# anisanazim/Movie-Recommendation-Engine

Measured on AMD Instinct MI355X. Metric: item embeddings/sec + top-K ANN queries/sec, ML-25M d=256, 1/2/4/8 GPU, higher is better.
Workload: dtype f64 cdf / f32 features / fp4 sign planes (exact integer Hamming); 1 GPU; SYN-25M (ML-25M-shaped: U=162541 M=59047 R=25000095), F=128 H=256 d=256, 2 GCN layers, W=100 L=2 T=10, LSH 512-bit, 10000 queries K=11, rng=numpy (the reference's np.random MT19937 stream generated on device: neighbour ids bit-exact with the reference CPU path); global_items=59047, queries=10000, parallelism=item-shard x1

## Files before the change

include/pinsage_hip.h:

```cpp
#ifndef PINSAGE_HIP_H
#define PINSAGE_HIP_H

#include <stddef.h>
#include <stdint.h>

#ifdef __cplusplus
extern "C" {
#endif

#define PS_OK 0
#define PS_EINVAL (-1)
#define PS_ELAUNCH (-2)
#define PS_EWORKSPACE (-3)
#define PS_EUNSUPPORTED (-4)

#define PS_RNG_STREAM 0
#define PS_RNG_PHILOX 1
#define PS_RNG_STREAM_RAW 2

#define PS_RNG_STREAM_WALKS 3

#define PS_WALK_HALF_BUCKETS 0x100

typedef void *ps_stream_t;

int ps_abi_version(void);
const char *ps_error_string(int code);

size_t ps_csr_build_workspace_bytes(int64_t E, int64_t V);
int ps_csr_build(const int64_t *src, const int64_t *dst, const float *w, int64_t E, int64_t V,
                 int64_t *rowptr, int32_t *col, double *wsorted,
                 void *workspace, size_t workspace_bytes, ps_stream_t stream);

int ps_cdf_build(const int64_t *rowptr, const double *wsorted, int64_t V, double *cdf, ps_stream_t stream);

int ps_guide_build(const int64_t *rowptr, const double *cdf, int64_t V, uint32_t *nodeinfo, int32_t *guide,
                   ps_stream_t stream);

int ps_pack_edges(const int32_t *col, const double *cdf, const int32_t *guide, int64_t E, void *packed,
                  ps_stream_t stream);

int ps_bucket_build(const int64_t *rowptr, const int32_t *col, const double *cdf, const int32_t *guide, int64_t V,
                    int64_t E, void *buckets, ps_stream_t stream);

int ps_bucket_build_half(const int64_t *rowptr, const int32_t *col, const double *cdf, const int32_t *guide, int64_t V,
                         int64_t E, void *buckets, ps_stream_t stream);

int ps_dest_info_build(const int32_t *col, const uint32_t *nodeinfo, int64_t E, int64_t V, void *dest_info, ps_stream_t stream);

int ps_graph_stats(const int64_t *rowptr, const int32_t *col, int64_t E, int64_t V, int64_t *flags,
                   ps_stream_t stream);

int ps_walk_sample(const int64_t *rowptr, const int32_t *col, const double *cdf, int64_t V,
                   const int64_t *starts, int64_t B, int W, int L, int T,
                   int rng_mode, const double *uniforms, const int64_t *uoff,
                   uint64_t seed, uint32_t call, const uint32_t *nodeinfo, const int32_t *guide,
                   const void *packed, const void *buckets, const void *dest_info,
                   int32_t *ids, int32_t *counts, int32_t *nvalid, ps_stream_t stream);

int ps_walk_sample_layers(const int64_t *rowptr, const int32_t *col, const double *cdf, int64_t V,
                          const int64_t *starts, int64_t B, int W, int L, int T,
                          int rng_mode, const double *uniforms, const int64_t *uoff, int64_t layer_stride,
                          uint64_t seed, uint32_t call, const uint32_t *nodeinfo, const int32_t *guide,
                          const void *packed, const void *buckets, const void *dest_info, int layers,
                          int32_t *ids, int32_t *counts, int32_t *nvalid, ps_stream_t stream);

int ps_walk_paths(const int64_t *rowptr, const int32_t *col, const double *cdf, int64_t V,
                  const int64_t *starts, int64_t B, int L, int rng_mode, const double *uniforms,
                  const int64_t *uoff, uint64_t seed, uint32_t call, int walk_mod,
                  const uint32_t *nodeinfo, const int32_t *guide, int32_t *paths, ps_stream_t stream);

int ps_uniform_offsets(const int64_t *rowptr, int64_t V, const int64_t *starts, int64_t B, int W, int L,
                       int64_t *uoff, int64_t *total, ps_stream_t stream);

int ps_mt19937_chunk_log2(void);
int ps_mt19937_window_shift(void);
int ps_mt19937_raw_stream(const uint32_t *state_in, int pos_in, int64_t n, uint32_t *raw, uint32_t *state_out,
                          int32_t *pos_out, const uint32_t *jump_polys, int jump_levels, const uint32_t *radix_polys,
                          int radix_levels, const uint32_t *window_polys, int n_window, const int64_t *ranges,
                          int n_ranges, void *workspace, size_t workspace_bytes, ps_stream_t stream);
size_t ps_mt19937_workspace_bytes(int64_t skip, int64_t n);
int ps_mt19937_random_sample(const uint32_t *state_in, int pos_in, int64_t skip, int64_t n, double *out,
                             uint32_t *state_out, int32_t *pos_out, const uint32_t *jump_polys, int jump_levels,
                             const uint32_t *radix_polys, int radix_levels, const uint32_t *window_polys, int n_window,
                             void *workspace, size_t workspace_bytes, ps_stream_t stream);

int ps_importance_pool(const float *x, int64_t N, int H, const int32_t *ids, const int32_t *counts,
                       const float *wts, const int32_t *nvalid, int64_t B, int T, int64_t max_idx,
                       int renorm, float *out, ps_stream_t stream);

#define PS_RELU 1
#define PS_L2NORM 2
#define PS_WPERM 4
int ps_permute_k(const float *W, int64_t rows, int K, int ld, float *out, ps_stream_t stream);
int ps_linear(const float *x, int64_t M, int K, const float *W, int ldw, const float *b, int N,
              const float *x2, int K2, const float *W2, int ldw2, int flags, float *y, ps_stream_t stream);

size_t ps_gcn_layer_workspace_bytes(int64_t M, int H);
int ps_gcn_layer(const float *x, int64_t M, int K, const float *W, int ldw, const float *b, int N, const float *h_full,
                 int64_t n_full, int H, const int32_t *ids, const int32_t *counts, const float *wts, const int32_t *nvalid,
                 int T, int64_t max_idx, int renorm, const float *W2, int ldw2, int flags, float *y, void *workspace,
                 size_t workspace_bytes, ps_stream_t stream);

int ps_lsh_encode(const float *x, int64_t N, int D, const float *A, int nbits, uint8_t *codes, int flags, ps_stream_t stream);

size_t ps_hamming_topk_workspace_bytes(int64_t nq, int64_t N, int cs, int k);
int ps_hamming_topk(const uint8_t *qcodes, int64_t nq, const uint8_t *codes, int64_t N, int cs, int k,
                    int64_t id_offset, int32_t *dist, int64_t *ids,
                    void *workspace, size_t workspace_bytes, ps_stream_t stream);

size_t ps_lsh_planes_bytes(int64_t n, int cs);
int ps_lsh_expand(const uint8_t *codes, int64_t n, int cs, void *planes, ps_stream_t stream);
size_t ps_hamming_topk_mfma_workspace_bytes(int64_t nq, int64_t N, int cs, int k);
int ps_hamming_topk_mfma(const void *qplanes, int64_t nq, const void *dbplanes, int64_t N, int cs, int k,
                         int64_t id_offset, int32_t *dist, int64_t *ids,
                         void *workspace, size_t workspace_bytes, ps_stream_t stream);
int ps_hamming_topk_mfma_codes(const uint8_t *qcodes, int64_t nq, const void *dbplanes, int64_t N, int cs, int k,
                               int64_t id_offset, int32_t *dist, int64_t *ids,
                               void *workspace, size_t workspace_bytes, ps_stream_t stream);

int ps_topk_merge(const int32_t *dist_in, const int64_t *ids_in, int P, int64_t nq, int k,
                  int32_t *dist, int64_t *ids, ps_stream_t stream);
int ps_topk_merge_strided(const int32_t *dist_in, int64_t dist_stride, const int64_t *ids_in, int64_t ids_stride,
                          int P, int64_t nq, int k, int32_t *dist, int64_t *ids, ps_stream_t stream);

size_t ps_dot_topk_workspace_bytes(int64_t nq, int64_t N, int D, int k);
int ps_dot_topk(const float *E, int64_t N, int D, const int64_t *qidx, int64_t nq, int k, int exclude_self,
                float *vals, int64_t *ids, void *workspace, size_t workspace_bytes, ps_stream_t stream);

int ps_row_dot(const float *A, int64_t nA, const float *B, int64_t nB, int D, const int64_t *ia, const int64_t *ib, int64_t n,
               float *out, ps_stream_t stream);
int ps_rank_count(const float *E, int64_t N, int D, int64_t id_offset, const float *Q, int64_t nq, const float *thr,
                  const int64_t *tid, int64_t *count, ps_stream_t stream);

size_t ps_l2_topk_workspace_bytes(int64_t nq, int64_t N, int D, int k);
int ps_l2_topk(const float *X, int64_t N, int D, const float *Q, int64_t nq, int k, const int32_t *assign,
               const uint32_t *probe, int words, float *dist, int64_t *ids, void *workspace,
               size_t workspace_bytes, ps_stream_t stream);

size_t ps_ivf_topk_workspace_bytes(int64_t nq, int64_t N, int D, int k, int nlist, int nprobe, int64_t max_list);
int ps_ivf_topk(const float *X, int64_t N, int D, const int64_t *list_ptr, int nlist, int64_t max_list,
                const int64_t *item_ids, const float *Q, int64_t nq, const int32_t *probes, int nprobe, int k,
                float *dist, int64_t *ids, void *workspace, size_t workspace_bytes, ps_stream_t stream);

int ps_spmm_csr(const int64_t *rowptr, const int32_t *col, const float *val, const float *x, int64_t N, int H,
                int64_t V, int64_t E, float *out, ps_stream_t stream);

#define PS_COOC_WINDOW 512
typedef struct {
    int32_t a, b, count, window;
} ps_cooc_record;
size_t ps_cooc_planes_bytes(int64_t U, int64_t M, int max_mult);
int ps_cooc_planes(const int32_t *user, const int32_t *item, const int32_t *mult, int64_t n, int64_t U, int64_t M,
                   int max_mult, void *planes, size_t planes_bytes, int64_t *item_stats, int32_t *max_seen, ps_stream_t stream);
int ps_cooc_pairs(const void *planes, int64_t U, int64_t M, int max_mult, int64_t max_sq, const int64_t *item_stats, int64_t thr,
                  ps_cooc_record *records, int64_t capacity, int64_t *count, int64_t *h_count, ps_stream_t stream);
int ps_cooc_keys(const ps_cooc_record *records, int64_t n, int64_t U, int64_t M, const int64_t *iptr, const int32_t *iuser,
                 const int32_t *imult, const int64_t *uptr, const int32_t *uitem, const int32_t *upos, int64_t R,
                 int64_t *keys, ps_stream_t stream);
int ps_cooc_emit(const ps_cooc_record *records, const int64_t *perm, int64_t n, int64_t *edge_index, float *edge_weight,
                 ps_stream_t stream);

#define PS_HN_PER_QUERY 1
#define PS_HN_EXCLUDE_DIAG 2
#define PS_LOSS_SHARED 0
#define PS_LOSS_PER_QUERY 1
#define PS_LOSS_BATCH_HARD 2
int ps_hardest_negative(const float *Q, int64_t B, int D, const float *X, int64_t N, int flags, uint64_t *best, float *sim,
                        int64_t *idx, ps_stream_t stream);
int ps_margin_loss(const float *Q, const float *P, int64_t B, int D, const uint64_t *best, float margin, float *row_loss,
                   int64_t *idx, uint8_t *active, float *loss, ps_stream_t stream);
int ps_margin_loss_bwd(const float *Q, const float *P, const float *X, int64_t B, int64_t N, int D, int mode, const int64_t *idx,
                       const uint8_t *active, const float *grad_out, float *dQ, float *dP, float *dX, ps_stream_t stream);

#ifdef __cplusplus
}
#endif
#endif
```

movie-recommendation-engine_amd/pinsage_hip/dense.py:

```python
from __future__ import annotations

import os

import torch

from . import native as nv


def _rowmajor(w):
    if w.dtype != torch.float32:
        raise TypeError("fp32 expected")
    if w.dim() != 2:
        raise ValueError("2-D matrix expected")
    if w.stride(1) != 1 or w.stride(0) < w.size(1):
        w = w.contiguous()
    return w, int(w.stride(0)) if w.size(0) > 1 else max(int(w.stride(0)), int(w.size(1)))


def _require_cuda(*tensors):
    for t in tensors:
        if t is not None and not t.is_cuda:
            raise nv.NativeError("libpinsage_hip takes device (HBM) tensors; got a CPU tensor (no CPU fallback)")


def _ptr_view(t):
    if t is None:
        return nv.C.c_void_p(0)
    if not t.is_cuda:
        raise nv.NativeError("device tensor expected")
    return nv.C.c_void_p(t.data_ptr())


class StagedWeight:
    __slots__ = ("t", "shape")

    def __init__(self, t):
        self.t = t
        self.shape = t.shape

    def size(self, i):
        return self.t.size(i)


def stage_weight(W):
    if isinstance(W, StagedWeight) or W is None:
        return W
    _require_cuda(W)
    if W.dim() != 2 or W.dtype != torch.float32 or int(W.size(1)) % 32 != 0:
        return W
    Wk, ld = _rowmajor(W)
    out = torch.empty((int(Wk.size(0)), int(Wk.size(1))), dtype=torch.float32, device=W.device)
    with torch.cuda.device(W.device):
        nv.call("ps_permute_k", _ptr_view(Wk), nv.i64(int(Wk.size(0))), nv.i32(int(Wk.size(1))), nv.i32(ld), nv.ptr(out), nv.stream())
    return StagedWeight(out)


def linear(x, W, b=None, x2=None, W2=None, relu=False, l2norm=False):
    staged = isinstance(W, StagedWeight)
    if x2 is not None and isinstance(W2, StagedWeight) != staged:
        raise ValueError("W and W2 must both be staged or both plain")
    if staged:
        W, W2 = W.t, (W2.t if W2 is not None else None)
    _require_cuda(x, W, b, x2, W2)
    x = x.contiguous()
    if x.dtype != torch.float32:
        raise TypeError("fp32 expected")
    M, K = int(x.size(0)), int(x.size(1))
    Wk, ldw = _rowmajor(W)
    N = int(Wk.size(0))
    if int(Wk.size(1)) != K:
        raise ValueError(f"shape mismatch: x [{M},{K}] vs W {tuple(Wk.shape)}")
    K2, ldw2, W2k = 0, 0, None
    if x2 is not None:
        x2 = x2.contiguous()
        W2k, ldw2 = _rowmajor(W2)
        K2 = int(x2.size(1))
        if int(W2k.size(1)) != K2 or int(W2k.size(0)) != N or int(x2.size(0)) != M:
            raise ValueError("shape mismatch in the second operand pair")
    if b is not None:
        b = b.contiguous()
    y = torch.empty((M, N), dtype=torch.float32, device=x.device)
    flags = (nv.PS_RELU if relu else 0) | (nv.PS_L2NORM if l2norm else 0) | (nv.PS_WPERM if staged else 0)
    with torch.cuda.device(x.device):
        nv.call("ps_linear", nv.ptr(x), nv.i64(M), nv.i32(K), _ptr_view(Wk), nv.i32(ldw), nv.ptr(b), nv.i32(N),
                                    nv.ptr(x2), nv.i32(K2), _ptr_view(W2k), nv.i32(ldw2), nv.i32(flags), nv.ptr(y),
                                    nv.stream())
    return y


def gcn_layer(x, W, b, h_full, ids, counts, nvalid, W2, wts=None, max_idx=None, renorm=True, relu=True, l2norm=True):
    from . import sampling
    staged = isinstance(W, StagedWeight)
    if isinstance(W2, StagedWeight) != staged:
        raise ValueError("W and W2 must both be staged or both plain")
    Wm, W2m = (W.t, W2.t) if staged else (W, W2)
    _require_cuda(x, Wm, b, h_full, W2m, ids, counts, wts, nvalid)
    x, h_full = x.contiguous(), h_full.contiguous()
    if x.dtype != torch.float32 or h_full.dtype != torch.float32:
        raise TypeError("fp32 expected")
    M, K = int(x.size(0)), int(x.size(1))
    n_full, H = int(h_full.size(0)), int(h_full.size(1))
    Wk, ldw = _rowmajor(Wm)
    W2k, ldw2 = _rowmajor(W2m)
    N = int(Wk.size(0))
    if int(Wk.size(1)) != K or int(W2k.size(1)) != H or int(W2k.size(0)) != N or int(ids.size(0)) != M:
        raise ValueError("shape mismatch")
    T = int(ids.size(1))
    if max_idx is None:
        max_idx = n_full - 1
    if b is not None:
        b = b.contiguous()
    ids, nvalid = ids.contiguous(), nvalid.contiguous()
    counts = counts.contiguous() if counts is not None else None
    wts = wts.contiguous() if wts is not None else None
    flags = (nv.PS_RELU if relu else 0) | (nv.PS_L2NORM if l2norm else 0) | (nv.PS_WPERM if staged else 0)
    L = nv.lib()
    wsb = int(L.ps_gcn_layer_workspace_bytes(nv.i64(M), nv.i32(H)))
    if wsb > 0:
        y = torch.empty((M, N), dtype=torch.float32, device=x.device)
        ws = torch.empty((wsb,), dtype=torch.uint8, device=x.device)
        with torch.cuda.device(x.device):
            rc = L.ps_gcn_layer(nv.ptr(x), nv.i64(M), nv.i32(K), _ptr_view(Wk), nv.i32(ldw), nv.ptr(b), nv.i32(N), nv.ptr(h_full),
                                nv.i64(n_full), nv.i32(H), nv.ptr(ids), nv.ptr(counts), nv.ptr(wts), nv.ptr(nvalid), nv.i32(T),
                                nv.i64(int(max_idx)), nv.i32(int(renorm)), _ptr_view(W2k), nv.i32(ldw2), nv.i32(flags), nv.ptr(y),
                                nv.ptr(ws), nv.C.c_size_t(wsb), nv.stream())
        if rc != nv.PS_EUNSUPPORTED:
            nv.check(rc, "ps_gcn_layer")
            return y
    h_neigh = sampling.importance_pool(h_full, ids=ids, counts=counts, wts=wts, nvalid=nvalid, max_idx=max_idx, renorm=renorm)
    return linear(x, W, b, x2=h_neigh, W2=W2, relu=relu, l2norm=l2norm)


def lsh_encode(x, A):
    staged = isinstance(A, StagedWeight)
    if staged:
        A = A.t
    _require_cuda(x, A)
    x = x.contiguous()
    A = A.contiguous()
    n, d = int(x.size(0)), int(x.size(1))
    nbits = int(A.size(0))
    if int(A.size(1)) != d:
        raise ValueError("projection matrix must be [nbits, dim]")
    codes = torch.empty((n, nbits // 8), dtype=torch.uint8, device=x.device)
    with torch.cuda.device(x.device):
        nv.call("ps_lsh_encode", nv.ptr(x), nv.i64(n), nv.i32(d), nv.ptr(A), nv.i32(nbits), nv.ptr(codes),
                                        nv.i32(nv.PS_WPERM if staged else 0), nv.stream())
    return codes


HAMMING_MAX_K = 64


def lsh_expand(codes):
    _require_cuda(codes)
    codes = codes.contiguous()
    n, cs = int(codes.size(0)), int(codes.size(1))
    nb = int(nv.lib().ps_lsh_planes_bytes(nv.i64(n), nv.i32(cs)))
    if nb == 0:
        return None
    planes = torch.empty(nb, dtype=torch.uint8, device=codes.device)
    with torch.cuda.device(codes.device):
        nv.call("ps_lsh_expand", nv.ptr(codes), nv.i64(n), nv.i32(cs), nv.ptr(planes), nv.stream())
    return planes


def hamming_mfma_supported(nq, N, cs, k):
    return int(nv.lib().ps_hamming_topk_mfma_workspace_bytes(nv.i64(nq), nv.i64(N), nv.i32(cs), nv.i32(k))) > 0


def hamming_topk(qcodes, codes, k, id_offset=0, planes=None, use_mfma=True, out=None):
    _require_cuda(qcodes, codes)
    qcodes = qcodes.contiguous()
    codes = codes.contiguous()
    nq, cs = int(qcodes.size(0)), int(qcodes.size(1))
    N = int(codes.size(0))
    if out is not None:
        dist, ids = out
        if (tuple(dist.shape) != (nq, k) or tuple(ids.shape) != (nq, k) or dist.dtype != torch.int32
                or ids.dtype != torch.int64 or not dist.is_contiguous() or not ids.is_contiguous()):
            raise ValueError("out must be contiguous (int32 [nq, k], int64 [nq, k])")
    if k > HAMMING_MAX_K or cs > 128 or (cs & (cs - 1)) != 0 or cs % 4 != 0:
        d, i = _hamming_topk_large_k(qcodes, codes, k, id_offset)
        if out is None:
            return d, i
        dist.copy_(d)
        ids.copy_(i)
        return dist, ids
    if out is None:
        dist = torch.empty((nq, k), dtype=torch.int32, device=qcodes.device)
        ids = torch.empty((nq, k), dtype=torch.int64, device=qcodes.device)
    L = nv.lib()
    if use_mfma and planes is not None:
        wsb = int(L.ps_hamming_topk_mfma_workspace_bytes(nv.i64(nq), nv.i64(N), nv.i32(cs), nv.i32(k)))
        if wsb > 0:
            ws = torch.empty(wsb, dtype=torch.uint8, device=qcodes.device)
            with torch.cuda.device(qcodes.device):
                nv.call("ps_hamming_topk_mfma_codes", nv.ptr(qcodes), nv.i64(nq), nv.ptr(planes), nv.i64(N), nv.i32(cs),
                        nv.i32(k), nv.i64(id_offset), nv.ptr(dist), nv.ptr(ids), nv.ptr(ws), nv.C.c_size_t(wsb),
                        nv.stream())
            return dist, ids
    wsb = int(L.ps_hamming_topk_workspace_bytes(nv.i64(nq), nv.i64(N), nv.i32(cs), nv.i32(k)))
    ws = torch.empty(wsb, dtype=torch.uint8, device=qcodes.device)
    with torch.cuda.device(qcodes.device):
        nv.call("ps_hamming_topk", nv.ptr(qcodes), nv.i64(nq), nv.ptr(codes) if N else nv.C.c_void_p(0), nv.i64(N),
                                   nv.i32(cs), nv.i32(k), nv.i64(id_offset), nv.ptr(dist), nv.ptr(ids), nv.ptr(ws),
                                   nv.C.c_size_t(wsb), nv.stream())
    return dist, ids


LARGE_K_SIGN_BYTES = 8 << 30


def _signs(codes):
    shifts = torch.arange(8, device=codes.device, dtype=torch.uint8)
    bits = (codes.unsqueeze(-1) >> shifts) & 1
    return bits.reshape(codes.size(0), -1).to(torch.float32) * 2.0 - 1.0


def _hamming_topk_large_k(qcodes, codes, k, id_offset):
    N, nbits = int(codes.size(0)), int(codes.size(1)) * 8
    if N * nbits * 4 > LARGE_K_SIGN_BYTES:
        raise ValueError(f"LSH search with k = {k} > {HAMMING_MAX_K} expands the code table to floats "
                         f"({N * nbits * 4 / 2 ** 30:.1f} GiB here, limit {LARGE_K_SIGN_BYTES >> 30} GiB): split the table or the request")
    d2, ids = l2_topk(_signs(codes), _signs(qcodes), k)
    missing = ids < 0
    dist = torch.where(missing, torch.full_like(d2, 0.0), d2 * 0.25).round().to(torch.int32)
    dist[missing] = 0x7fffffff
    ids = torch.where(missing, ids, ids + int(id_offset))
    return dist, ids


def topk_merge(dist_in, ids_in):
    dist_in = dist_in.contiguous()
    ids_in = ids_in.contiguous()
    P, nq, k = [int(v) for v in dist_in.shape]
    dist = torch.empty((nq, k), dtype=torch.int32, device=dist_in.device)
    ids = torch.empty((nq, k), dtype=torch.int64, device=dist_in.device)
    with torch.cuda.device(dist_in.device):
        nv.call("ps_topk_merge", nv.ptr(dist_in), nv.ptr(ids_in), nv.i32(P), nv.i64(nq), nv.i32(k), nv.ptr(dist),
                                        nv.ptr(ids), nv.stream())
    return dist, ids


def topk_merge_records(records, nq, k):
    if records.dtype != torch.uint8 or records.dim() != 2 or not records.is_contiguous():
        raise ValueError("records must be a contiguous uint8 [P, record_bytes] tensor")
    P, rec = int(records.size(0)), int(records.size(1))
    n = int(nq) * int(k)
    if rec < 12 * n or rec % 8 != 0:
        raise ValueError("record too short or not 8-byte aligned")
    dist = torch.empty((nq, k), dtype=torch.int32, device=records.device)
    ids = torch.empty((nq, k), dtype=torch.int64, device=records.device)
    base = records.data_ptr()
    with torch.cuda.device(records.device):
        nv.call("ps_topk_merge_strided", nv.C.c_void_p(base + 8 * n), nv.i64(rec // 4), nv.C.c_void_p(base), nv.i64(rec // 8),
                nv.i32(P), nv.i64(int(nq)), nv.i32(int(k)), nv.ptr(dist), nv.ptr(ids), nv.stream())
    return dist, ids


def dot_topk(E, qidx, k, exclude_self=True):
    E = E.contiguous()
    qidx = qidx.to(device=E.device, dtype=torch.int64).contiguous()
    N, D = int(E.size(0)), int(E.size(1))
    nq = int(qidx.numel())
    if k < 1:
        raise ValueError(f"k must be positive, got {k}")
    vals = torch.empty((nq, k), dtype=torch.float32, device=E.device)
    ids = torch.empty((nq, k), dtype=torch.int64, device=E.device)
    L = nv.lib()
    wsb = int(L.ps_dot_topk_workspace_bytes(nv.i64(nq), nv.i64(N), nv.i32(D), nv.i32(k)))
    ws = torch.empty(wsb, dtype=torch.uint8, device=E.device)
    with torch.cuda.device(E.device):
        nv.call("ps_dot_topk", nv.ptr(E), nv.i64(N), nv.i32(D), nv.ptr(qidx), nv.i64(nq), nv.i32(k),
                               nv.i32(int(exclude_self)), nv.ptr(vals), nv.ptr(ids), nv.ptr(ws), nv.C.c_size_t(wsb),
                               nv.stream())
    return vals, ids


def _fp32_rows(E):
    _require_cuda(E)
    if E.dtype != torch.float32 or E.dim() != 2:
        raise TypeError("fp32 [N, D] matrix expected")
    return E.contiguous()


def row_dot(A, ia, B, ib):
    A, B = _fp32_rows(A), _fp32_rows(B)
    if int(A.size(1)) != int(B.size(1)):
        raise ValueError(f"shape mismatch: A {tuple(A.shape)} vs B {tuple(B.shape)}")
    ia = ia.to(device=A.device, dtype=torch.int64).contiguous()
    ib = ib.to(device=A.device, dtype=torch.int64).contiguous()
    if ia.numel() != ib.numel():
        raise ValueError("ia and ib must have the same length")
    out = torch.empty(int(ia.numel()), dtype=torch.float32, device=A.device)
    with torch.cuda.device(A.device):
        nv.call("ps_row_dot", nv.ptr(A), nv.i64(int(A.size(0))), nv.ptr(B), nv.i64(int(B.size(0))), nv.i32(int(A.size(1))),
# ... 192 lines not shown
```

movie-recommendation-engine_amd/pinsage_hip/native.py:

```python
from __future__ import annotations

import ctypes as C
import os

import torch

_HERE = os.path.dirname(os.path.abspath(__file__))
SO_PATH = os.environ.get("PS_HIP_LIB") or os.path.join(_HERE, "libpinsage_hip.so")
_lib = None

PS_RNG_STREAM = 0
PS_RNG_PHILOX = 1
PS_RNG_STREAM_RAW = 2
PS_RNG_STREAM_WALKS = 3
PS_WALK_HALF_BUCKETS = 0x100
PS_RELU = 1
PS_L2NORM = 2
PS_WPERM = 4
PS_HN_PER_QUERY, PS_HN_EXCLUDE_DIAG = 1, 2
PS_LOSS_SHARED, PS_LOSS_PER_QUERY, PS_LOSS_BATCH_HARD = 0, 1, 2
PS_OK, PS_EINVAL, PS_ELAUNCH, PS_EWORKSPACE, PS_EUNSUPPORTED = 0, -1, -2, -3, -4


class LibraryMissing(RuntimeError):
    pass


class NativeError(RuntimeError):
    pass


SYMBOLS = [
    "ps_abi_version", "ps_error_string", "ps_csr_build_workspace_bytes", "ps_csr_build", "ps_cdf_build",
    "ps_guide_build", "ps_pack_edges", "ps_bucket_build", "ps_bucket_build_half", "ps_dest_info_build", "ps_graph_stats", "ps_walk_sample", "ps_walk_sample_layers", "ps_walk_paths", "ps_uniform_offsets", "ps_mt19937_window_shift", "ps_mt19937_workspace_bytes", "ps_mt19937_chunk_log2", "ps_mt19937_random_sample", "ps_mt19937_raw_stream",
    "ps_importance_pool", "ps_permute_k", "ps_linear", "ps_gcn_layer_workspace_bytes", "ps_gcn_layer", "ps_lsh_encode", "ps_hamming_topk_workspace_bytes", "ps_hamming_topk",
    "ps_lsh_planes_bytes", "ps_lsh_expand", "ps_hamming_topk_mfma_workspace_bytes", "ps_hamming_topk_mfma", "ps_hamming_topk_mfma_codes",
    "ps_topk_merge", "ps_topk_merge_strided", "ps_dot_topk_workspace_bytes", "ps_dot_topk", "ps_row_dot", "ps_rank_count", "ps_l2_topk_workspace_bytes", "ps_l2_topk", "ps_ivf_topk_workspace_bytes", "ps_ivf_topk", "ps_spmm_csr",
    "ps_cooc_planes_bytes", "ps_cooc_planes", "ps_cooc_pairs", "ps_cooc_keys", "ps_cooc_emit",
    "ps_hardest_negative", "ps_margin_loss", "ps_margin_loss_bwd",
]


def have_lib() -> bool:
    return os.path.exists(SO_PATH)


def lib():
    global _lib
    if _lib is None:
        if not have_lib():
            raise LibraryMissing(
                f"{SO_PATH} not found: build it with `python -c 'import __graft_entry__ as g; g.build()'` "
                "(hipcc --offload-arch=gfx950).  There is no CPU fallback for the PinSage hot path.")
        _lib = C.CDLL(SO_PATH)
        _lib.ps_error_string.restype = C.c_char_p
        for name in ("ps_csr_build_workspace_bytes", "ps_hamming_topk_workspace_bytes", "ps_dot_topk_workspace_bytes",
                     "ps_l2_topk_workspace_bytes", "ps_ivf_topk_workspace_bytes", "ps_mt19937_workspace_bytes", "ps_lsh_planes_bytes",
                     "ps_hamming_topk_mfma_workspace_bytes", "ps_gcn_layer_workspace_bytes", "ps_cooc_planes_bytes"):
            if hasattr(_lib, name):
                getattr(_lib, name).restype = C.c_size_t
    return _lib


def check(rc: int, what: str):
    if rc != 0:
        raise NativeError(f"{what}: {lib().ps_error_string(rc).decode()} (code {rc})")


class KernelTimer:

    def __init__(self):
        self.events = []

    def summary(self):
        torch.cuda.synchronize()
        out = {}
        for name, a, b in self.events:
            d = out.setdefault(name, {"launches": 0, "ms": 0.0})
            d["launches"] += 1
            d["ms"] += a.elapsed_time(b)
        for d in out.values():
            d["avg_ms"] = d["ms"] / d["launches"]
        return out


_timer = None


def set_timer(t):
    global _timer
    _timer = t


def call(name, *args):
    fn = getattr(lib(), name)
    if _timer is None:
        rc = fn(*args)
    else:
        a, b = torch.cuda.Event(enable_timing=True), torch.cuda.Event(enable_timing=True)
        a.record()
        rc = fn(*args)
        b.record()
        _timer.events.append((name, a, b))
    check(rc, name)


def ptr(t):
    if t is None:
        return C.c_void_p(0)
    if not t.is_cuda:
        raise NativeError("libpinsage_hip takes device (HBM) pointers; got a CPU tensor")
    if not t.is_contiguous():
        raise NativeError("tensor must be contiguous")
    return C.c_void_p(t.data_ptr())


_raw_stream = getattr(torch._C, "_cuda_getCurrentRawStream", None)
_get_device = getattr(torch._C, "_cuda_getDevice", None)


def stream():
    if _raw_stream is not None and _get_device is not None:
        return C.c_void_p(_raw_stream(_get_device()))
    return C.c_void_p(torch.cuda.current_stream().cuda_stream)


def require_gpu():
    if not torch.cuda.is_available():
        raise NativeError("the PinSage hot path needs an MI355X (torch.cuda is not available); "
                          "there is no CPU fallback")
    lib()
    return torch.device("cuda", torch.cuda.current_device())


i64 = C.c_int64
i32 = C.c_int
u64 = C.c_uint64
u32 = C.c_uint32
```

movie-recommendation-engine_amd/pinsage_hip/shard.py:

```python
from __future__ import annotations

import os

import torch
import torch.distributed as dist

from . import dense, sampling


def shard_range(M, rank, world):
    chunk = (M + world - 1) // world
    lo = min(rank * chunk, M)
    return lo, min(lo + chunk, M), chunk


def _backend(group):
    return dist.get_backend(group) if dist.is_initialized() else None


class _Gather:

    def __init__(self, out, work=None, dev=None):
        self.out, self.work, self.dev = out, work, dev

    def wait(self):
        if self.work is not None:
            self.work.wait()
        return self.out if self.dev is None else self.out.to(self.dev)


class Comm:

    def __init__(self, group=None, standin=None):
        self.group = group
        self.standin = standin
        if standin is not None:
            self.rank, self.world = int(standin[0]), int(standin[1])
        elif dist.is_initialized():
            self.rank, self.world = dist.get_rank(group), dist.get_world_size(group)
        else:
            self.rank, self.world = 0, 1
        self._bufs = {}

    def _buf(self, kind, tag, shape, dtype, device, zero=False):
        key = (kind, tag, tuple(shape), dtype, str(device))
        b = self._bufs.get(key)
        if b is None:
            b = (torch.zeros if zero else torch.empty)(tuple(shape), dtype=dtype, device=device)
            self._bufs[key] = b
        return b

    def gather_rows_async(self, t, chunk, tag="rows"):
        if self.world == 1:
            return _Gather(t)
        rest = tuple(t.shape[1:])
        if self.standin is not None:
            key = ("recv", tag, (self.world * chunk,) + rest, t.dtype, str(t.device))
            fresh = key not in self._bufs
            out = self._buf("recv", tag, (self.world * chunk,) + rest, t.dtype, t.device, zero=True)
            for r in (range(self.world) if fresh else (self.rank,)):
                out[r * chunk: r * chunk + t.size(0)].copy_(t)
            return _Gather(out)
        if t.size(0) == chunk and t.is_contiguous():
            src = t
        else:
            src = self._buf("send", tag, (chunk,) + rest, t.dtype, t.device, zero=True)
            src[: t.size(0)].copy_(t)
        if _backend(self.group) == "gloo" and src.is_cuda:
            out = torch.empty((self.world * chunk,) + rest, dtype=t.dtype)
            dist.all_gather_into_tensor(out, src.cpu().contiguous(), group=self.group)
            return _Gather(out, dev=t.device)
        out = self._buf("recv", tag, (self.world * chunk,) + rest, t.dtype, src.device)
        work = dist.all_gather_into_tensor(out, src, group=self.group, async_op=True)
        return _Gather(out, work)

    def gather_rows(self, t, chunk, tag="rows"):
        return self.gather_rows_async(t, chunk, tag).wait()


def all_gather_rows_async(t, chunk, group=None):
    c = Comm(group)
    return c.gather_rows_async(t, chunk)


def all_gather_rows(t, chunk, group=None):
    return all_gather_rows_async(t, chunk, group).wait()


def fused_self_update(ops, P, i, H):
    Ws, bs = P[f"convs.{i}.lin_self.weight"], P[f"convs.{i}.lin_self.bias"]
    Wu, bu = P[f"convs.{i}.lin_update.weight"], P[f"convs.{i}.lin_update.bias"]
    Wu1 = Wu[:, :H].contiguous()
    W1 = ops.linear(Wu1, Ws.t().contiguous(), None)
    b1 = ops.linear(bs.reshape(1, -1).contiguous(), Wu1, bu).reshape(-1)
    return W1, b1


class HipOps:

    def sample(self, sampler, nodes, T, shard=None):
        if shard is not None and getattr(sampler, "rng", None) == "numpy":
            M, lo = shard
            all_nodes = torch.arange(M, dtype=torch.int64, device=nodes.device)
            return sampler.sample_batch(nodes, T, stream_nodes=(all_nodes, lo))
        return sampler.sample_batch(nodes, T)

    def sample_layers(self, sampler, lo, hi, T, layers, shard=None):
        stream = None
        if shard is not None and getattr(sampler, "rng", None) == "numpy":
            stream = (range(shard[0]), shard[1])
        return sampler.sample_batches(range(lo, hi), T, layers, stream_nodes=stream, defer_state=True)

    def finish(self):
        dense.finish_rng_state()

    def pool(self, h_full, batch, max_idx):
        return sampling.importance_pool(h_full, batch, max_idx=max_idx)

    def linear(self, x, W, b, x2=None, W2=None, relu=False, l2norm=False):
        return dense.linear(x, W, b, x2=x2, W2=W2, relu=relu, l2norm=l2norm)

    def gcn_layer(self, x, W, b, h_full, batch, max_idx, W2):
        return dense.gcn_layer(x, W, b, h_full, batch.ids, batch.counts, batch.nvalid, W2, max_idx=max_idx)

    def lsh_encode(self, x, A):
        return dense.lsh_encode(x, A)

    def stage_weight(self, W):
        return dense.stage_weight(W)

    def lsh_planes(self, codes):
        return dense.lsh_expand(codes)

    def hamming_topk(self, q, codes, k, id_offset, planes=None, out=None):
        return dense.hamming_topk(q, codes, k, id_offset=id_offset, planes=planes, out=out)

    def topk_merge(self, d, i):
        return dense.topk_merge(d, i)

    def topk_merge_records(self, records, nq, k):
        return dense.topk_merge_records(records, nq, k)


class ShardedPinSage:

    def __init__(self, params, num_layers, sampler, num_items, ops=None, group=None, standin=None):
        self.P = params
        self.num_layers = num_layers
        self.sampler = sampler
        self.M = int(num_items)
        self.ops = ops if ops is not None else HipOps()
        self.group = group
        self.comm = Comm(group, standin=standin)
        self.rank, self.world = self.comm.rank, self.comm.world
        self.lo, self.hi, self.chunk = shard_range(self.M, self.rank, self.world)
        self._nodes = {}
        self.overlap_sampling = False
        self.overlap_input_proj = os.environ.get("PS_OVERLAP_INPUT_PROJ") == "1"
        self.fuse_self = True
        self._streams = {}
        self._fused = {}
        self._staged = {}

    def refresh_weights(self, params=None):
        if params is not None:
            self.P = params
        self._fused.clear()
        self._staged.clear()

    def _fused_layer(self, i, H):
        if i not in self._fused:
            self._fused[i] = fused_self_update(self.ops, self.P, i, H)
        return self._fused[i]

    def _w(self, key, W):
        if not hasattr(self.ops, "stage_weight"):
            return W
        t = self._staged.get(key)
        if t is None:
            t = self._staged[key] = self.ops.stage_weight(W)
        return t

    def _side_stream(self, dev):
        key = str(dev)
        if key not in self._streams:
            self._streams[key] = torch.cuda.Stream(device=dev)
        return self._streams[key]

    def _sample(self, nodes, T, shard):
        try:
            return self.ops.sample(self.sampler, nodes, T, shard)
        except TypeError:
            return self.ops.sample(self.sampler, nodes, T)

    def embed(self, x_local, T, x_full=None):
        try:
            return self._embed(x_local, T, x_full)
        finally:
            if hasattr(self.ops, "finish"):
                self.ops.finish()

    def _embed(self, x_local, T, x_full=None):
        ops, P = self.ops, self.P
        dev = x_local.device
        fused = (not (self.overlap_sampling and x_local.is_cuda)) and hasattr(ops, "sample_layers") \
            and hasattr(self.sampler, "sample_batches")
        nodes = None
        if not fused:
            nodes = self._nodes.get(str(dev))
            if nodes is None:
                nodes = self._nodes[str(dev)] = torch.arange(self.lo, self.hi, dtype=torch.int64, device=dev)
        shard = (self.M, self.lo) if self.world > 1 else None
        side = self._side_stream(dev) if (self.overlap_sampling and x_local.is_cuda) else None
        batches, ready = [], []
        early_h = None
        if (self.overlap_input_proj and fused and x_local.is_cuda and getattr(self.sampler, "rng", None) == "numpy"
                and not (x_full is not None and self.world > 1)):
            main = torch.cuda.current_stream(dev)
            aux = self._side_stream(dev)
            aux.wait_stream(main)
            with torch.cuda.stream(aux):
                early_h = ops.linear(x_local, self._w("in", P["input_proj.weight"]), P["input_proj.bias"], relu=True)
                early_ready = aux.record_event()
            early_h.record_stream(main)
        if fused:
            batches = list(ops.sample_layers(self.sampler, self.lo, self.hi, T, self.num_layers, shard))
        elif side is not None:
            main = torch.cuda.current_stream(dev)
            side.wait_stream(main)
            with torch.cuda.stream(side):
                for _ in range(self.num_layers):
                    b = self._sample(nodes, T, shard)
                    for t in (b.ids, b.counts, b.nvalid):
                        t.record_stream(main)
                    batches.append(b)
                    ready.append(side.record_event())
        else:
            batches.append(self._sample(nodes, T, shard))
        if early_h is not None:
            torch.cuda.current_stream(dev).wait_event(early_ready)
        if x_full is not None and self.world > 1:
            h_all = ops.linear(x_full, self._w("in", P["input_proj.weight"]), P["input_proj.bias"], relu=True)
            h = h_all[self.lo:self.hi]
            pending = _Gather(h_all)
        else:
            h = early_h if early_h is not None else ops.linear(x_local, self._w("in", P["input_proj.weight"]), P["input_proj.bias"], relu=True)
            pending = self.comm.gather_rows_async(h, self.chunk, "h")
        for i in range(self.num_layers):
            if side is None and not fused and i + 1 < self.num_layers:
                batches.append(self._sample(nodes, T, shard))
            H = h.size(1)
            Wu = P[f"convs.{i}.lin_update.weight"]
            if self.fuse_self:
                W1, b1 = self._fused_layer(i, H)
                a_in = h
            else:
                a_in = ops.linear(h, P[f"convs.{i}.lin_self.weight"], P[f"convs.{i}.lin_self.bias"])
                W1, b1 = Wu[:, :H], P[f"convs.{i}.lin_update.bias"]
            h_full = pending.wait()
            if side is not None:
                torch.cuda.current_stream(dev).wait_event(ready[i])
            if self.fuse_self and hasattr(ops, "gcn_layer"):
                h = ops.gcn_layer(a_in, self._w(("l1", i), W1), b1, h_full, batches[i], self.M - 1, self._w(("l2", i), Wu[:, H:]))
            else:
                h_neigh = ops.pool(h_full, batches[i], self.M - 1)
                h = ops.linear(a_in, self._w(("l1", i), W1), b1, x2=h_neigh, W2=self._w(("l2", i), Wu[:, H:]), relu=True, l2norm=True)
            if i + 1 < self.num_layers:
                pending = self.comm.gather_rows_async(h, self.chunk, "h")
        return ops.linear(h, self._w("out", P["output_proj.weight"]), P["output_proj.bias"], l2norm=True)

    def _staged_A(self, A):
        if not hasattr(self.ops, "stage_weight") or not isinstance(A, torch.Tensor):
            return A
        ent = self._staged.get("A")
        if ent is None or ent[0] is not A or ent[1] != A._version:
            ent = self._staged["A"] = (A, A._version, self.ops.stage_weight(A))
        return ent[2]

    REPLICATE_CODES_BYTES = 64 << 20

    def build_index(self, emb_local, A):
        self.A = A
        self.codes = self.ops.lsh_encode(emb_local, self._staged_A(A))
        self.codes_all = None
        if self.world > 1 and self.M * int(self.codes.size(1)) <= self.REPLICATE_CODES_BYTES:
            self.codes_all = self.comm.gather_rows(self.codes, self.chunk, "codes")[: self.M]
        scanned = self.codes_all if self.codes_all is not None else self.codes
        self.planes = self.ops.lsh_planes(scanned) if hasattr(self.ops, "lsh_planes") else None
        return self.codes

    def search(self, q_local, k):
        ops = self.ops
        qc = ops.lsh_encode(q_local, self._staged_A(self.A))
        nq_local = qc.size(0)
        planes = getattr(self, "planes", None)
        if self.world > 1 and getattr(self, "codes_all", None) is not None:
            n = nq_local * k
            rec = (12 * n + 15) // 16 * 16
            mine = self.comm._buf("res", "mine", (1, rec), torch.uint8, qc.device, zero=True)
            ids_v = mine[0, : 8 * n].view(torch.int64).view(nq_local, k)
            dist_v = mine[0, 8 * n: 12 * n].view(torch.int32).view(nq_local, k)
            try:
                ops.hamming_topk(qc, self.codes_all, k, 0, planes=planes, out=(dist_v, ids_v))
            except TypeError:
                d, i = ops.hamming_topk(qc, self.codes_all, k, 0)
                dist_v.copy_(d)
                ids_v.copy_(i)
            allr = self.comm.gather_rows(mine, 1, "res")
            P_ = self.world
            return (allr[:, 8 * n: 12 * n].view(torch.int32).reshape(P_ * nq_local, k),
                    allr[:, : 8 * n].view(torch.int64).reshape(P_ * nq_local, k))
        qc_all = self.comm.gather_rows(qc, nq_local, "qcodes")
        if self.world == 1:
            return (ops.hamming_topk(qc_all, self.codes, k, self.lo, planes=planes) if planes is not None
                    else ops.hamming_topk(qc_all, self.codes, k, self.lo))
        nq = qc_all.size(0)
        n = nq * k
        rec = (12 * n + 15) // 16 * 16
        mine = self.comm._buf("cand", "mine", (1, rec), torch.uint8, qc_all.device, zero=True)
        ids_v = mine[0, : 8 * n].view(torch.int64).view(nq, k)
        dist_v = mine[0, 8 * n: 12 * n].view(torch.int32).view(nq, k)
        try:
            ops.hamming_topk(qc_all, self.codes, k, self.lo, planes=planes, out=(dist_v, ids_v))
        except TypeError:
            d, i = ops.hamming_topk(qc_all, self.codes, k, self.lo)
            dist_v.copy_(d)
            ids_v.copy_(i)
        allc = self.comm.gather_rows(mine, 1, "cand")
        if hasattr(ops, "topk_merge_records"):
            return ops.topk_merge_records(allc, nq, k)
        d_all = torch.stack([allc[p, 8 * n: 12 * n].view(torch.int32).view(nq, k) for p in range(self.world)])
        i_all = torch.stack([allc[p, : 8 * n].view(torch.int64).view(nq, k) for p in range(self.world)])
        return ops.topk_merge(d_all, i_all)
```

Before: 44.56 million items/s.

## Add bf16x3 MFMA LSH encode with exact fp32 fallback for near-zero projections

Adds a filtered LSH encode kernel that computes the item-by-hyperplane projections with split bf16 (hi/lo) MFMA products, then decides each sign bit only when the value clears a norm-based error bound. Undecided bits are collected in a shared list and recomputed in exact fp32 chained FMA order, so the codes stay bit-exact with the old path. If the list overflows, the block falls back to fp32 MFMA. The projection matrix is pre-split into bf16 planes at staging time. This trades the cost of the fp32 projection for extra staging, shared-memory use and a per-bit check, aiming to speed up both index build and query encoding.

```diff
diff --git a/include/pinsage_hip.h b/include/pinsage_hip.h
--- a/include/pinsage_hip.h
+++ b/include/pinsage_hip.h
@@ -104,6 +104,11 @@
 
 int ps_lsh_encode(const float *x, int64_t N, int D, const float *A, int nbits, uint8_t *codes, int flags, ps_stream_t stream);
 
+size_t ps_lsh_split_bytes(int nbits, int D);
+int ps_lsh_split(const float *A, int nbits, int D, void *planes, ps_stream_t stream);
+int ps_lsh_encode_filtered(const float *x, int64_t N, int D, const float *A, const void *planes, int nbits, uint8_t *codes,
+                           int flags, uint64_t *stats, ps_stream_t stream);
+
 size_t ps_hamming_topk_workspace_bytes(int64_t nq, int64_t N, int cs, int k);
 int ps_hamming_topk(const uint8_t *qcodes, int64_t nq, const uint8_t *codes, int64_t N, int cs, int k,
                     int64_t id_offset, int32_t *dist, int64_t *ids,
diff --git a/movie-recommendation-engine_amd/csrc/lsh_filter.hip b/movie-recommendation-engine_amd/csrc/lsh_filter.hip
--- /dev/null
+++ b/movie-recommendation-engine_amd/csrc/lsh_filter.hip
@@ -0,0 +1,286 @@
+#include "ps_common.h"
+
+#ifndef PS_LSH_FILTER_DEBUG
+#define PS_LSH_FILTER_DEBUG 0
+#endif
+
+namespace {
+
+typedef float f32x16 __attribute__((ext_vector_type(16)));
+typedef float f32x4 __attribute__((ext_vector_type(4)));
+typedef uint32_t u32x4 __attribute__((ext_vector_type(4)));
+typedef __bf16 bf16x8 __attribute__((ext_vector_type(8)));
+
+constexpr float LSH_C = 0x1p-12f;
+constexpr float LSH_INFLATE = 1.0f + 0x1p-10f;
+constexpr float LSH_NORM_LO = 0x1p-40f, LSH_NORM_HI = 0x1p40f;
+constexpr int LSH_BM = 128;
+constexpr int LSH_LIST = 4096;
+constexpr int LSH_MAX_WORDS = 32;
+constexpr int64_t LSH_MIN_ROWS = 2048;
+
+#if PS_LSH_FILTER_DEBUG
+__device__ float *ps_lsh_filter_dump_ptr;
+#endif
+
+__device__ __forceinline__ uint32_t bf16_bits(float v) {
+    const uint32_t b = __float_as_uint(v);
+    return (b + 0x7fffu + ((b >> 16) & 1u)) >> 16;
+}
+__device__ __forceinline__ void split8(const f32x4 a, const f32x4 b, u32x4 &hi, u32x4 &lo) {
+    const float v[8] = {a[0], a[1], a[2], a[3], b[0], b[1], b[2], b[3]};
+    uint32_t h[8], l[8];
+#pragma unroll
+    for (int j = 0; j < 8; ++j) {
+        h[j] = bf16_bits(v[j]);
+        l[j] = bf16_bits(v[j] - __uint_as_float(h[j] << 16));
+    }
+#pragma unroll
+    for (int j = 0; j < 4; ++j) {
+        hi[j] = h[2 * j] | (h[2 * j + 1] << 16);
+        lo[j] = l[2 * j] | (l[2 * j + 1] << 16);
+    }
+}
+__device__ __forceinline__ float sumsq8(const f32x4 a, const f32x4 b, float s) {
+#pragma unroll
+    for (int j = 0; j < 4; ++j) s = fmaf(a[j], a[j], s);
+#pragma unroll
+    for (int j = 0; j < 4; ++j) s = fmaf(b[j], b[j], s);
+    return s;
+}
+__device__ __forceinline__ float norm_bound(float ss) {
+    const float n = sqrtf(ss) * LSH_INFLATE;
+    return (n >= LSH_NORM_LO && n <= LSH_NORM_HI) ? n : __builtin_inff();
+}
+
+__host__ __device__ constexpr int lsh_ksteps(int D) { return D <= 64 ? 4 : D <= 128 ? 8 : 16; }
+
+__global__ void lsh_split_kernel(const float *__restrict__ A, int nbits, int D, int KS, u32x4 *__restrict__ planes, float *__restrict__ na) {
+    const int lane = threadIdx.x & 63, r = lane & 31, h = lane >> 5;
+    const int item = blockIdx.x * (blockDim.x >> 6) + (threadIdx.x >> 6);
+    if (item >= (nbits / 32) * KS) return;
+    const int ct = item / KS, s = item % KS, k = 16 * s + 8 * h;
+    const float *row = A + (int64_t)(ct * 32 + r) * D;
+    f32x4 a = {0.f, 0.f, 0.f, 0.f}, b = a;
+    if (k < D) {
+        a = *reinterpret_cast<const f32x4 *>(row + k);
+        b = *reinterpret_cast<const f32x4 *>(row + k + 4);
+    }
+    u32x4 hi, lo;
+    split8(a, b, hi, lo);
+    planes[((int64_t)item * 2) * 64 + lane] = hi;
+    planes[((int64_t)item * 2 + 1) * 64 + lane] = lo;
+    if (s == 0 && h == 0) {
+        float ss = 0.f;
+        for (int kk = 0; kk < D; kk += 8)
+            ss = sumsq8(*reinterpret_cast<const f32x4 *>(row + kk), *reinterpret_cast<const f32x4 *>(row + kk + 4), ss);
+        na[ct * 32 + r] = norm_bound(ss);
+    }
+}
+
+__device__ __forceinline__ float chain8(const f32x4 x0, const f32x4 x1, const f32x4 p, const f32x4 q, bool wp, float s) {
+    if (wp) {
+        s = fmaf(x0[0], p[0], s); s = fmaf(x0[1], q[0], s); s = fmaf(x0[2], p[1], s); s = fmaf(x0[3], q[1], s);
+        s = fmaf(x1[0], p[2], s); s = fmaf(x1[1], q[2], s); s = fmaf(x1[2], p[3], s); s = fmaf(x1[3], q[3], s);
+    } else {
+        s = fmaf(x0[0], p[0], s); s = fmaf(x0[1], p[1], s); s = fmaf(x0[2], p[2], s); s = fmaf(x0[3], p[3], s);
+        s = fmaf(x1[0], q[0], s); s = fmaf(x1[1], q[1], s); s = fmaf(x1[2], q[2], s); s = fmaf(x1[3], q[3], s);
+    }
+    return s;
+}
+__device__ __forceinline__ float exact_chain(const float *__restrict__ x, const float *__restrict__ a, int D, bool wp) {
+    float s = 0.f;
+    for (int k = 0; k < D; k += 32) {
+        f32x4 xv[8], av[8];
+#pragma unroll
+        for (int j = 0; j < 8; ++j) {
+            xv[j] = *reinterpret_cast<const f32x4 *>(x + k + 4 * j);
+            av[j] = *reinterpret_cast<const f32x4 *>(a + k + 4 * j);
+        }
+#pragma unroll
+        for (int j = 0; j < 4; ++j) s = chain8(xv[2 * j], xv[2 * j + 1], av[2 * j], av[2 * j + 1], wp, s);
+    }
+    return s;
+}
+
+template <int KS>
+__global__ __launch_bounds__(256, 2) void lsh_filter_kernel(const float *__restrict__ x, int64_t N, int D, const float *__restrict__ A,
+                                                            const u32x4 *__restrict__ planes, const float *__restrict__ na, int nbits,
+                                                            uint32_t *__restrict__ codes, int wperm, unsigned long long *stats) {
+    __shared__ u32x4 sB[KS * 2 * 64];
+    __shared__ uint32_t sCodes[LSH_BM * LSH_MAX_WORDS];
+    __shared__ uint32_t sList[LSH_LIST];
+    __shared__ float sTau[LSH_BM];
+    __shared__ int sCount;
+    const int tid = threadIdx.x, lane = tid & 63, wv = tid >> 6, r = lane & 31, h = lane >> 5;
+    const int words = nbits >> 5;
+    const int64_t m0 = (int64_t)blockIdx.x * LSH_BM;
+    const int rows = N - m0 < LSH_BM ? (int)(N - m0) : LSH_BM;
+    const bool wp = wperm != 0;
+
+    const int rowl = wv * 32 + r;
+    const bool rok = rowl < rows;
+    const float *xr = x + (m0 + (rok ? rowl : 0)) * D;
+    u32x4 xh[KS], xl[KS];
+    float ss = 0.f;
+#pragma unroll
+    for (int s = 0; s < KS; ++s) {
+        const int k = 16 * s + 8 * h;
+        f32x4 a = {0.f, 0.f, 0.f, 0.f}, b = a;
+        if (k < D) {
+            a = *reinterpret_cast<const f32x4 *>(xr + k);
+            b = *reinterpret_cast<const f32x4 *>(xr + k + 4);
+        }
+        ss = sumsq8(a, b, ss);
+        split8(a, b, xh[s], xl[s]);
+    }
+    ss += __shfl_xor(ss, 32);
+    if (h == 0) sTau[rowl] = rok ? LSH_C * norm_bound(ss) : -1.f;
+    if (tid == 0) sCount = 0;
+    __syncthreads();
+
+    constexpr int NST = KS * 2 * 64 / 256;
+    u32x4 st[NST];
+#pragma unroll
+    for (int q = 0; q < NST; ++q) st[q] = planes[tid + 256 * q];
+    for (int ct = 0; ct < words; ++ct) {
+        if (ct > 0) __syncthreads();
+#pragma unroll
+        for (int q = 0; q < NST; ++q) sB[tid + 256 * q] = st[q];
+        __syncthreads();
+        {
+            const u32x4 *np = planes + (int64_t)(ct + 1 < words ? ct + 1 : ct) * KS * 2 * 64;
+#pragma unroll
+            for (int q = 0; q < NST; ++q) st[q] = np[tid + 256 * q];
+        }
+        const u32x4 *bp = sB + lane;
+        f32x16 accM, accC;
+#pragma unroll
+        for (int g = 0; g < 16; ++g) accM[g] = accC[g] = 0.f;
+#pragma unroll
+        for (int s = 0; s < KS; ++s) {
+            const bf16x8 bh = __builtin_bit_cast(bf16x8, bp[(2 * s) * 64]), bl = __builtin_bit_cast(bf16x8, bp[(2 * s + 1) * 64]);
+            const bf16x8 ah = __builtin_bit_cast(bf16x8, xh[s]), al = __builtin_bit_cast(bf16x8, xl[s]);
+            accM = __builtin_amdgcn_mfma_f32_32x32x16_bf16(ah, bh, accM, 0, 0, 0);
+            accC = __builtin_amdgcn_mfma_f32_32x32x16_bf16(ah, bl, accC, 0, 0, 0);
+            accC = __builtin_amdgcn_mfma_f32_32x32x16_bf16(al, bh, accC, 0, 0, 0);
+        }
+        const float nac = na[ct * 32 + r];
+#pragma unroll
+        for (int g = 0; g < 16; ++g) {
+            const float f = accM[g] + accC[g];
+            const int row = wv * 32 + (g & 3) + 8 * (g >> 2) + 4 * h;
+#if PS_LSH_FILTER_DEBUG
+            if (ps_lsh_filter_dump_ptr != nullptr && row < rows) ps_lsh_filter_dump_ptr[(m0 + row) * nbits + ct * 32 + r] = f;
+#endif
+            const bool decided = fabsf(f) > sTau[row] * nac;
+            const uint64_t bits = __ballot(decided && f >= 0.f);
+            if (r == 0) sCodes[row * words + ct] = h ? (uint32_t)(bits >> 32) : (uint32_t)bits;
+            if (__ballot(!decided) != 0ull) {
+                if (!decided) {
+                    const int i = atomicAdd(&sCount, 1);
+                    if (i < LSH_LIST) sList[i] = ((uint32_t)row << 16) | (uint32_t)(ct * 32 + r);
+                }
+            }
+        }
+    }
+    __syncthreads();
+    const int count = sCount;
+    if (count <= LSH_LIST) {
+        for (int i = tid; i < count; i += 256) {
+            const uint32_t e = sList[i];
+            const int row = (int)(e >> 16), col = (int)(e & 0xffffu);
+            const float s = exact_chain(x + (m0 + row) * D, A + (int64_t)col * D, D, wp);
+            if (s >= 0.f) atomicOr(&sCodes[row * words + (col >> 5)], 1u << (col & 31));
+        }
+    } else {
+        for (int ct = 0; ct < words; ++ct) {
+            const float *ar = A + (int64_t)(ct * 32 + r) * D;
+            f32x16 acc;
+#pragma unroll
+            for (int g = 0; g < 16; ++g) acc[g] = 0.f;
+            for (int k = 0; k < D; k += 32) {
+                f32x4 xq[8], aq[8];
+#pragma unroll
+                for (int j = 0; j < 8; ++j) xq[j] = *reinterpret_cast<const f32x4 *>(xr + k + 4 * j);
+#pragma unroll
+                for (int j = 0; j < 8; ++j)
+                    aq[j] = wp ? *reinterpret_cast<const f32x4 *>(ar + k + 8 * (j >> 1) + 4 * h) : *reinterpret_cast<const f32x4 *>(ar + k + 4 * j);
+#pragma unroll
+                for (int j = 0; j < 4; ++j) {
+                    const f32x4 x0 = xq[2 * j], x1 = xq[2 * j + 1], a0 = aq[2 * j], a1 = aq[2 * j + 1];
+                    const f32x4 xv = h ? f32x4{x0[1], x0[3], x1[1], x1[3]} : f32x4{x0[0], x0[2], x1[0], x1[2]};
+                    const f32x4 av = wp ? a0 : h ? f32x4{a0[1], a0[3], a1[1], a1[3]} : f32x4{a0[0], a0[2], a1[0], a1[2]};
+#pragma unroll
+                    for (int t = 0; t < 4; ++t) acc = __builtin_amdgcn_mfma_f32_32x32x2f32(xv[t], av[t], acc, 0, 0, 0);
+                }
+            }
+#pragma unroll
+            for (int g = 0; g < 16; ++g) {
+                const uint64_t bits = __ballot(acc[g] >= 0.f);
+                const int row = wv * 32 + (g & 3) + 8 * (g >> 2) + 4 * h;
+                if (r == 0) sCodes[row * words + ct] = h ? (uint32_t)(bits >> 32) : (uint32_t)bits;
+            }
+        }
+    }
+    __syncthreads();
+    uint32_t *dst = codes + m0 * words;
+    for (int i = tid; i < rows * words; i += 256) dst[i] = sCodes[i];
+    if (stats != nullptr && tid == 0) {
+        if (count <= LSH_LIST) { if (count) atomicAdd(stats, (unsigned long long)count); }
+        else atomicAdd(stats + 1, 1ull);
+    }
+}
+
+bool lsh_filter_shape(int D, int nbits) {
+    return D > 0 && D % 32 == 0 && D <= 256 && nbits > 0 && nbits % 32 == 0 && nbits <= 32 * LSH_MAX_WORDS;
+}
+
+}
+
+#if PS_LSH_FILTER_DEBUG
+extern "C" int ps_debug_lsh_filter_dump(float *buf) {
+    return (int)hipMemcpyToSymbol(HIP_SYMBOL(ps_lsh_filter_dump_ptr), &buf, sizeof buf);
+}
+#endif
+
+extern "C" size_t ps_lsh_split_bytes(int nbits, int D) {
+    if (!lsh_filter_shape(D, nbits)) return 0;
+    return (size_t)nbits * lsh_ksteps(D) * 16 * 2 * 2 + (size_t)nbits * sizeof(float);
+}
+
+extern "C" int ps_lsh_split(const float *A, int nbits, int D, void *planes, ps_stream_t stream) {
+    if (nbits <= 0 || D <= 0) return PS_EINVAL;
+    if (!lsh_filter_shape(D, nbits)) return PS_EUNSUPPORTED;
+    if (!A || !planes) return PS_EINVAL;
+    if (reinterpret_cast<size_t>(A) % 16 != 0 || reinterpret_cast<size_t>(planes) % 16 != 0) return PS_EUNSUPPORTED;
+    const int KS = lsh_ksteps(D), items = (nbits / 32) * KS;
+    float *na = reinterpret_cast<float *>(static_cast<char *>(planes) + (size_t)nbits * KS * 16 * 2 * 2);
+    hipLaunchKernelGGL(lsh_split_kernel, dim3((unsigned)ps_cdiv(items, 4)), dim3(256), 0, ps_stream(stream), A, nbits, D, KS,
+                       static_cast<u32x4 *>(planes), na);
+    PS_CHECK_LAUNCH();
+    return PS_OK;
+}
+
+extern "C" int ps_lsh_encode_filtered(const float *x, int64_t N, int D, const float *A, const void *planes, int nbits, uint8_t *codes,
+                                      int flags, uint64_t *stats, ps_stream_t stream) {
+    if (N < 0 || D <= 0 || nbits <= 0 || (flags & ~PS_WPERM)) return PS_EINVAL;
+    if (!lsh_filter_shape(D, nbits) || N < LSH_MIN_ROWS || N > (int64_t)0x7fffffff * LSH_BM) return PS_EUNSUPPORTED;
+    if (!x || !A || !planes || !codes || reinterpret_cast<size_t>(stats) % 8 != 0) return PS_EINVAL;
+    if (reinterpret_cast<size_t>(x) % 16 != 0 || reinterpret_cast<size_t>(A) % 16 != 0 || reinterpret_cast<size_t>(planes) % 16 != 0 ||
+        reinterpret_cast<size_t>(codes) % 4 != 0) return PS_EUNSUPPORTED;
+    const char *fe = getenv("PS_LSH_FILTER");
+    if (fe && atoi(fe) == 0) return PS_EUNSUPPORTED;
+    const int KS = lsh_ksteps(D);
+    const u32x4 *pl = static_cast<const u32x4 *>(planes);
+    const float *na = reinterpret_cast<const float *>(static_cast<const char *>(planes) + (size_t)nbits * KS * 16 * 2 * 2);
+    uint32_t *c32 = reinterpret_cast<uint32_t *>(codes);
+    unsigned long long *st = reinterpret_cast<unsigned long long *>(stats);
+    const dim3 grid((unsigned)ps_cdiv(N, LSH_BM)), block(256);
+    hipStream_t hs = ps_stream(stream);
+    if (KS == 4) hipLaunchKernelGGL(lsh_filter_kernel<4>, grid, block, 0, hs, x, N, D, A, pl, na, nbits, c32, flags & PS_WPERM, st);
+    else if (KS == 8) hipLaunchKernelGGL(lsh_filter_kernel<8>, grid, block, 0, hs, x, N, D, A, pl, na, nbits, c32, flags & PS_WPERM, st);
+    else hipLaunchKernelGGL(lsh_filter_kernel<16>, grid, block, 0, hs, x, N, D, A, pl, na, nbits, c32, flags & PS_WPERM, st);
+    PS_CHECK_LAUNCH();
+    return PS_OK;
+}
diff --git a/movie-recommendation-engine_amd/pinsage_hip/dense.py b/movie-recommendation-engine_amd/pinsage_hip/dense.py
--- a/movie-recommendation-engine_amd/pinsage_hip/dense.py
+++ b/movie-recommendation-engine_amd/pinsage_hip/dense.py
@@ -32,17 +32,32 @@
 
 
 class StagedWeight:
-    __slots__ = ("t", "shape")
-
-    def __init__(self, t):
+    __slots__ = ("t", "shape", "planes", "plain")
+
+    def __init__(self, t, planes=None, plain=None):
         self.t = t
         self.shape = t.shape
+        self.planes = planes
+        self.plain = plain
 
     def size(self, i):
         return self.t.size(i)
 
 
-def stage_weight(W):
+def lsh_split(A):
+    _require_cuda(A)
+    A = A.contiguous()
+    nbits, d = int(A.size(0)), int(A.size(1))
+    nb = int(nv.lib().ps_lsh_split_bytes(nv.i32(nbits), nv.i32(d)))
+    if nb == 0 or A.dtype != torch.float32 or A.data_ptr() % 16 != 0:
+        return None
+    planes = torch.empty(nb, dtype=torch.uint8, device=A.device)
+    with torch.cuda.device(A.device):
+        nv.call("ps_lsh_split", nv.ptr(A), nv.i32(nbits), nv.i32(d), nv.ptr(planes), nv.stream())
+    return planes
+
+
+def stage_weight(W, lsh=False):
     if isinstance(W, StagedWeight) or W is None:
         return W
     _require_cuda(W)
@@ -52,7 +67,7 @@
     out = torch.empty((int(Wk.size(0)), int(Wk.size(1))), dtype=torch.float32, device=W.device)
     with torch.cuda.device(W.device):
         nv.call("ps_permute_k", _ptr_view(Wk), nv.i64(int(Wk.size(0))), nv.i32(int(Wk.size(1))), nv.i32(ld), nv.ptr(out), nv.stream())
-    return StagedWeight(out)
+    return StagedWeight(out, lsh_split(Wk), Wk) if lsh else StagedWeight(out)
 
 
 def linear(x, W, b=None, x2=None, W2=None, relu=False, l2norm=False):
@@ -131,8 +146,11 @@
     return linear(x, W, b, x2=h_neigh, W2=W2, relu=relu, l2norm=l2norm)
 
 
-def lsh_encode(x, A):
+def lsh_encode(x, A, stats=None):
     staged = isinstance(A, StagedWeight)
+    planes = A.planes if staged else None
+    if staged and A.plain is not None and x.is_cuda and x.contiguous().data_ptr() % 16 != 0:
+        A, staged, planes = A.plain, False, None
     if staged:
         A = A.t
     _require_cuda(x, A)
@@ -143,6 +161,13 @@
     if int(A.size(1)) != d:
         raise ValueError("projection matrix must be [nbits, dim]")
     codes = torch.empty((n, nbits // 8), dtype=torch.uint8, device=x.device)
+    if planes is not None and x.dtype == torch.float32 and A.dtype == torch.float32:
+        with torch.cuda.device(x.device):
+            rc = nv.lib().ps_lsh_encode_filtered(nv.ptr(x), nv.i64(n), nv.i32(d), nv.ptr(A), nv.ptr(planes), nv.i32(nbits), nv.ptr(codes),
+                                                 nv.i32(nv.PS_WPERM), nv.ptr(stats), nv.stream())
+        if rc != nv.PS_EUNSUPPORTED:
+            nv.check(rc, "ps_lsh_encode_filtered")
+            return codes
     with torch.cuda.device(x.device):
         nv.call("ps_lsh_encode", nv.ptr(x), nv.i64(n), nv.i32(d), nv.ptr(A), nv.i32(nbits), nv.ptr(codes),
                                         nv.i32(nv.PS_WPERM if staged else 0), nv.stream())
diff --git a/movie-recommendation-engine_amd/pinsage_hip/native.py b/movie-recommendation-engine_amd/pinsage_hip/native.py
--- a/movie-recommendation-engine_amd/pinsage_hip/native.py
+++ b/movie-recommendation-engine_amd/pinsage_hip/native.py
@@ -33,7 +33,7 @@
 SYMBOLS = [
     "ps_abi_version", "ps_error_string", "ps_csr_build_workspace_bytes", "ps_csr_build", "ps_cdf_build",
     "ps_guide_build", "ps_pack_edges", "ps_bucket_build", "ps_bucket_build_half", "ps_dest_info_build", "ps_graph_stats", "ps_walk_sample", "ps_walk_sample_layers", "ps_walk_paths", "ps_uniform_offsets", "ps_mt19937_window_shift", "ps_mt19937_workspace_bytes", "ps_mt19937_chunk_log2", "ps_mt19937_random_sample", "ps_mt19937_raw_stream",
-    "ps_importance_pool", "ps_permute_k", "ps_linear", "ps_gcn_layer_workspace_bytes", "ps_gcn_layer", "ps_lsh_encode", "ps_hamming_topk_workspace_bytes", "ps_hamming_topk",
+    "ps_importance_pool", "ps_permute_k", "ps_linear", "ps_gcn_layer_workspace_bytes", "ps_gcn_layer", "ps_lsh_encode", "ps_lsh_split_bytes", "ps_lsh_split", "ps_lsh_encode_filtered", "ps_hamming_topk_workspace_bytes", "ps_hamming_topk",
     "ps_lsh_planes_bytes", "ps_lsh_expand", "ps_hamming_topk_mfma_workspace_bytes", "ps_hamming_topk_mfma", "ps_hamming_topk_mfma_codes",
     "ps_topk_merge", "ps_topk_merge_strided", "ps_dot_topk_workspace_bytes", "ps_dot_topk", "ps_row_dot", "ps_rank_count", "ps_l2_topk_workspace_bytes", "ps_l2_topk", "ps_ivf_topk_workspace_bytes", "ps_ivf_topk", "ps_spmm_csr",
     "ps_cooc_planes_bytes", "ps_cooc_planes", "ps_cooc_pairs", "ps_cooc_keys", "ps_cooc_emit",
@@ -56,7 +56,7 @@
         _lib.ps_error_string.restype = C.c_char_p
         for name in ("ps_csr_build_workspace_bytes", "ps_hamming_topk_workspace_bytes", "ps_dot_topk_workspace_bytes",
                      "ps_l2_topk_workspace_bytes", "ps_ivf_topk_workspace_bytes", "ps_mt19937_workspace_bytes", "ps_lsh_planes_bytes",
-                     "ps_hamming_topk_mfma_workspace_bytes", "ps_gcn_layer_workspace_bytes", "ps_cooc_planes_bytes"):
+                     "ps_hamming_topk_mfma_workspace_bytes", "ps_gcn_layer_workspace_bytes", "ps_cooc_planes_bytes", "ps_lsh_split_bytes"):
             if hasattr(_lib, name):
                 getattr(_lib, name).restype = C.c_size_t
     return _lib
diff --git a/movie-recommendation-engine_amd/pinsage_hip/shard.py b/movie-recommendation-engine_amd/pinsage_hip/shard.py
--- a/movie-recommendation-engine_amd/pinsage_hip/shard.py
+++ b/movie-recommendation-engine_amd/pinsage_hip/shard.py
@@ -126,8 +126,8 @@
     def lsh_encode(self, x, A):
         return dense.lsh_encode(x, A)
 
-    def stage_weight(self, W):
-        return dense.stage_weight(W)
+    def stage_weight(self, W, lsh=False):
+        return dense.stage_weight(W, lsh=lsh)
 
     def lsh_planes(self, codes):
         return dense.lsh_expand(codes)
@@ -274,7 +274,11 @@
             return A
         ent = self._staged.get("A")
         if ent is None or ent[0] is not A or ent[1] != A._version:
-            ent = self._staged["A"] = (A, A._version, self.ops.stage_weight(A))
+            try:
+                S = self.ops.stage_weight(A, lsh=True)
+            except TypeError:
+                S = self.ops.stage_weight(A)
+            ent = self._staged["A"] = (A, A._version, S)
         return ent[2]
 
     REPLICATE_CODES_BYTES = 64 << 20
```

Result: no change. 44.65 million items/s, median of 6 (+0.2%).
